# kdexd/virtex

Hardware: NVIDIA H100
Metric: image-caption pairs/sec bicaptioning R50-L1-H1024 (higher is better)
Workload: dtype bf16

## Files before the change

virtex_b200/csrc/gemm_tc.cu:

```cuda
#include <stdlib.h>
#include "ptx.cuh"
#include "vtx_common.cuh"
#include "../../include/virtex_b200.h"

#define KP_TAPS_W p.taps_w
#define KP_PAD p.pad
#define KP_NTAPS p.ntaps

namespace vtx {

constexpr int kBM = 128;
constexpr int kBK = 64;
constexpr int kMaxStages = 8;
constexpr int kABytes = kBM * kBK * 2;
constexpr int kSmemTotal = 232448;
constexpr int kCtrlBytes = 1024;
constexpr int kThreads = 384;
constexpr int kEpiThreads = 256;

struct FastDiv {
  uint32_t mul, shr;
};
__device__ __forceinline__ int fdiv(int x, const FastDiv& f) {
  return f.mul == 0u ? x : (int)(__umulhi((uint32_t)x, f.mul) >> f.shr);
// ... 18 lines not shown
  int bn;
  int a_mn, b_mn;
  int m_tiles, n_tiles, k_splits;
  int kb_total, kb_per_split;
  int mode;
  int cH, cW, cN, cpb;
  int lbw, lbh, lbn;
  int tiles_w, tiles_h;
  int out_f32, atomic, act;
  int stages, stage_bytes;
  int cbytes, nbuf;
  int res_tma;
  float alpha;
  void* D;
  long long ldd;
  const float* bias;
  int bias_pairs;
  const __nv_bfloat16* residual;
  long long ldr;
  const uint8_t* res_mask;
  float* stats;
  int taps_w, pad, ntaps;
  int cstride;
  FastDiv d_mn, d_nt, d_mt, d_tw, d_twh, d_cpb, d_taps;
  unsigned int* sched;
  unsigned int sched_base;
  int sched_chunk;
  int nt_major;
  const __nv_bfloat16* bnr_y;
  const float* bnr_bnp;
  const uint8_t* bnr_mask;
  long long bnr_ldy, bnr_sw, bnr_sh, bnr_sn;
  int vW, vH;
  int bnr_prefetch;
  int bnr;
  int trans_d;
  const float* col_scale;
  const float* col_shift;
};

__device__ __forceinline__ float gelu_erf(float x) { return 0.5f * x * (1.0f + erff(x * 0.70710678118654752f)); }

__device__ __forceinline__ void epi_bar(int id, int threads) {
  asm volatile("bar.sync %0, %1;" ::"r"(id), "r"(threads) : "memory");
}

__device__ __forceinline__ void decode_tile(const GemmKParams& p, int t, int& ks, int& mt, int& nt) {
  ks = fdiv(t, p.d_mn);
  const int rem = t - ks * (p.m_tiles * p.n_tiles);
  if (p.nt_major) {
    nt = fdiv(rem, p.d_mt);
    mt = rem - nt * p.m_tiles;
  } else {
    mt = fdiv(rem, p.d_nt);
    nt = rem - mt * p.n_tiles;
  }
}
__device__ __forceinline__ void tma_prefetch_l2_2d(const void* tmap, int c0, int c1) {
  asm volatile("cp.async.bulk.prefetch.tensor.2d.L2.global.tile [%0, {%1, %2}];" ::"l"(reinterpret_cast<uint64_t>(tmap)),
               "r"(c0), "r"(c1)
               : "memory");
}
__device__ __forceinline__ void tma_prefetch_l2_4d(const void* tmap, int c0, int c1, int c2, int c3) {
  asm volatile("cp.async.bulk.prefetch.tensor.4d.L2.global.tile [%0, {%1, %2, %3, %4}];" ::"l"(
                   reinterpret_cast<uint64_t>(tmap)),
               "r"(c0), "r"(c1), "r"(c2), "r"(c3)
               : "memory");
// ... 248 lines not shown
    }
    epi_bar(bar_id, epi_threads);
    if (et < p.bn && st_nt * p.bn + et < p.N) {
      float a = 0.f, b = 0.f;
      for (int g = 0; g < st_rgs; ++g) {
        const float2 v = *reinterpret_cast<const float2*>(scr + (g * p.bn + et) * 2);
        a += v.x;
        b += v.y;
      }
      if (p.bnr) b *= __ldg(p.bnr_bnp + p.N + st_nt * p.bn + et);
      atomicAdd(p.stats + st_nt * p.bn + et, a);
      atomicAdd(p.stats + p.N + st_nt * p.bn + et, b);
    }
    epi_bar(bar_id, epi_threads);
  };
  auto issue_residual = [&](int t_, int bi_) {
    int ks_, mt_, nt_;
    decode_tile(p, t_, ks_, mt_, nt_);
    const int nb_ = nt_ * p.bn;
    uint8_t* buf_ = cstage0 + (size_t)bi_ * p.cbytes;
    const int slabs = (min(p.bn, p.N - nb_) + 63) >> 6;
    mbar_arrive_expect_tx(&res_bar[bi_], (uint32_t)slabs * 16384u);
    for (int sl = 0; sl < slabs; ++sl) {
      if (p.mode & 1) {
        const int tn_ = fdiv(mt_, p.d_twh);
        const int rwh_ = mt_ - tn_ * (p.tiles_w * p.tiles_h);
        const int th_ = fdiv(rwh_, p.d_tw), tw_ = rwh_ - th_ * p.tiles_w;
        tma_load_4d(buf_ + sl * 16384, &tmR, &res_bar[bi_], nb_ + sl * 64, tw_ << p.lbw, th_ << p.lbh, tn_ << p.lbn);
      } else {
        tma_load_2d(buf_ + sl * 16384, &tmR, &res_bar[bi_], nb_ + sl * 64, mt_ * kBM);
      }
    }
  };
  float acc[NH * BN / 2];
  for (int it = 0;; ++it) {
    const int sit = PP ? 2 * it + wg : it;
    const int slot = sit & (kSched - 1);
    mbar_wait(&sch_full[slot], (sit / kSched) & 1);
    const unsigned long long tk = sch_tile[slot];
    const int t = (int)(uint32_t)tk;
    const int kpos = (int)(tk >> 32);
    mbar_arrive(&sch_empty[slot]);
    if (t >= total_tiles) break;
    int ks, mt, nt;
    decode_tile(p, t, ks, mt, nt);
    const int n_base = nt * p.bn;
    int tw = 0, th = 0, tn = 0;
    if (p.mode & 1) {
      tn = fdiv(mt, p.d_twh);
      const int r_wh = mt - tn * (p.tiles_w * p.tiles_h);
      th = fdiv(r_wh, p.d_tw);
      tw = r_wh - th * p.tiles_w;
    }
    const int cbi = PP ? wg : p.nbuf > 1 ? (it & 1) : 0;
    uint8_t* cbuf = cstage0 + (size_t)cbi * p.cbytes;
    if (staged) {
      if (p.bnr && p.res_tma) epi_bar(bar_id, epi_threads);
      if (et == 0) {
        if (!PP && p.nbuf > 1) tma_store_wait_read<1>();
        else tma_store_wait_read<0>();
      }
      const bool new_block = p.stats != nullptr && st_nt != nt;
      if (new_block && st_nt >= 0 && p.res_tma) {
        epi_bar(bar_id, epi_threads);
        flush_stats(cbuf);
      }
      if (et == 0) {
        if (p.res_tma) issue_residual(t, cbi);
        if (p.bnr && p.bnr_prefetch) {
          const int slabs = (min(p.bn, p.N - n_base) + 63) >> 6;
          for (int sl = 0; sl < slabs; ++sl) {
            if (p.mode & 1) tma_prefetch_l2_4d(&tmY, n_base + sl * 64, tw << p.lbw, th << p.lbh, tn << p.lbn);
            else tma_prefetch_l2_2d(&tmY, n_base + sl * 64, mt * kBM);
          }
        }
      }
      epi_bar(bar_id, epi_threads);
      if (new_block) {
        if (st_nt >= 0 && !p.res_tma) flush_stats(cbuf);
        st_nt = nt;
      }
    }

    {
      const int kb0 = ks * p.kb_per_split;
      const int kb1 = min(p.kb_total, kb0 + p.kb_per_split);
      const int stage = kpos % p.stages;
      const uint32_t phase = (uint32_t)(kpos / p.stages) & 1u;
      const uint32_t a_off = PP ? 0u : (uint32_t)wg * 8192u;
      uint64_t* order_next = nullptr;
      if (PP) {
        if (wg == 1) mbar_wait(&order_bar[1], (uint32_t)it & 1u);
        else if (it > 0) mbar_wait(&order_bar[0], (uint32_t)(it - 1) & 1u);
        order_next = &order_bar[wg ^ 1];
      }
      if (!p.a_mn && !p.b_mn)
        mma_tile<BN, NH, 0, 0>(acc, smem, p, kb0, kb1, a_off, full_bar, empty_bar, stage, phase, signal, order_next);
      else if (!p.a_mn)
        mma_tile<BN, NH, 0, 1>(acc, smem, p, kb0, kb1, a_off, full_bar, empty_bar, stage, phase, signal, order_next);
      else if (!p.b_mn)
        mma_tile<BN, NH, 1, 0>(acc, smem, p, kb0, kb1, a_off, full_bar, empty_bar, stage, phase, signal, order_next);
      else
        mma_tile<BN, NH, 1, 1>(acc, smem, p, kb0, kb1, a_off, full_bar, empty_bar, stage, phase, signal, order_next);
    }
    if (p.res_tma) {
      const int uses = PP ? it : p.nbuf > 1 ? (it >> 1) : it;
      mbar_wait(&res_bar[cbi], uses & 1);
    }
// ... 47 lines not shown
      const uint32_t srow = smem_u32(cbuf) + ((PP ? 0 : wg) * 64 + wl * 16 + (lane >> 2)) * 128 + q * 4;
      const int sw = lane >> 2;
      const int col0 = n_base + 2 * q;
#pragma unroll
      for (int j = 0; j < BN / 8; ++j) {
        const int col = col0 + 8 * j;
        const float2 b = col < p.N ? __ldg(reinterpret_cast<const float2*>(p.bias + col)) : make_float2(0.f, 0.f);
        const uint32_t sa = srow + (j >> 3) * 16384 + (((j & 7) ^ sw) << 4);
#pragma unroll
        for (int hh = 0; hh < 2 * NH; ++hh) {
          const float* accb = acc + (hh >> 1) * (BN / 2) + 4 * j + 2 * (hh & 1);
          sts32(sa + ((hh >> 1) * 64 + 8 * (hh & 1)) * 128, pack_bf16x2(accb[0] + b.x, accb[1] + b.y));
        }
      }
    } else if (plain || p.res_tma) {
#pragma unroll
      for (int hh = 0; hh < 2 * NH; ++hh) {
        const int hr = hh & 1;
        const float* accb = acc + (hh >> 1) * (BN / 2);
        const int r_in_tile = (PP ? (hh >> 1) : wg) * 64 + wl * 16 + (lane >> 2) + 8 * hr;
        const uint32_t srow = smem_u32(cbuf) + r_in_tile * 128 + q * 4;
        const int sw = r_in_tile & 7;
        if (plain) {
#pragma unroll
          for (int j = 0; j < BN / 8; ++j)
            sts32(srow + (j >> 3) * 16384 + (((j & 7) ^ sw) << 4), pack_bf16x2(accb[4 * j + 2 * hr], accb[4 * j + 2 * hr + 1]));
        } else if (p.res_mask == nullptr) {
#pragma unroll
          for (int j = 0; j < BN / 8; ++j) {
            const uint32_t sa = srow + (j >> 3) * 16384 + (((j & 7) ^ sw) << 4);
            sts32(sa, add_res_bf16x2(accb[4 * j + 2 * hr], accb[4 * j + 2 * hr + 1], lds32(sa)));
          }
        } else {
          const long long grow = tile_row(r_in_tile);
          uint32_t mword = 0u;
#pragma unroll
          for (int j = 0; j < BN / 8; ++j) {
            const int col = n_base + 8 * j + 2 * q;
            if ((j & 3) == 0)
              mword = (grow >= 0 && col < p.N)
                          ? __ldg(reinterpret_cast<const uint32_t*>(p.res_mask) + ((grow * p.N + col) >> 5)) : 0u;
            const uint32_t sa = srow + (j >> 3) * 16384 + (((j & 7) ^ sw) << 4);
            const uint32_t r = lds32(sa) & ((((mword >> (col & 31)) & 1u) ? 0x0000ffffu : 0u) |
                                            (((mword >> ((col & 31) + 1)) & 1u) ? 0xffff0000u : 0u));
            sts32(sa, add_res_bf16x2(accb[4 * j + 2 * hr], accb[4 * j + 2 * hr + 1], r));
          }
        }
      }
    } else if (f32_only) {
      float* const D = reinterpret_cast<float*>(p.D);
#pragma unroll
      for (int hh = 0; hh < 2 * NH; ++hh) {
        const int hr = hh & 1;
        const float* accb = acc + (hh >> 1) * (BN / 2);
        const int r_in_tile = (PP ? (hh >> 1) : wg) * 64 + wl * 16 + (lane >> 2) + 8 * hr;
        const long long grow = tile_row(r_in_tile);
        if (grow < 0) continue;
        if (p.trans_d) {
#pragma unroll
          for (int j = 0; j < BN / 8; ++j) {
            const int col = n_base + 8 * j + 2 * q;
            if (col >= p.N) continue;
            float* op = D + (long long)col * p.ldd + grow;
            atomicAdd(op, accb[4 * j + 2 * hr] * p.alpha);
            if (col + 1 < p.N) atomicAdd(op + p.ldd, accb[4 * j + 2 * hr + 1] * p.alpha);
          }
        } else if (p.atomic) {
#pragma unroll
          for (int j = 0; j < BN / 8; ++j) {
            const int col = n_base + 8 * j + 2 * q;
            if (col >= p.N) continue;
            float* op = D + grow * p.ldd + col;
            const float v0 = accb[4 * j + 2 * hr] * p.alpha, v1 = accb[4 * j + 2 * hr + 1] * p.alpha;
            if (col + 1 < p.N) red_add_v2(op, v0, v1);
// ... 50 lines not shown
          if (p.act == 1) {
            v0 = fmaxf(v0, 0.f);
            v1 = fmaxf(v1, 0.f);
          } else if (p.act == 2) {
            v0 = gelu_erf(v0);
            v1 = gelu_erf(v1);
          }
          if (staged) {
            sts32(sa, pack_bf16x2(v0, v1));
          } else if (grow >= 0) {
            float* D = reinterpret_cast<float*>(p.D);
            if (p.trans_d) {
              float* op = D + (long long)col * p.ldd + grow;
              atomicAdd(op, v0);
              if (two) atomicAdd(op + p.ldd, v1);
            } else {
              float* op = D + grow * p.ldd + col;
              if (p.atomic) {
                if (two) red_add_v2(op, v0, v1);
                else atomicAdd(op, v0);
              } else if (two) {
                *reinterpret_cast<float2*>(op) = make_float2(v0, v1);
              } else {
                op[0] = v0;
              }
            }
          }
        }
      }
    }

    const int bnr_r0 = srg * st_rpt;
    const int bnr_col = n_base + scg * 8;
    const bool bnr_on = p.bnr && st_on && bnr_col < p.N;
    auto bnr_load = [&](int rb, uint4* yv, uint32_t& mbits) {
      mbits = 0u;
#pragma unroll
      for (int r4 = 0; r4 < 4; ++r4) {
        const int r = bnr_r0 + rb + r4;
        uint32_t off, lin = 0;
        bool ok;
        if (p.mode & 1) {
          const int dw = r & ((1 << p.lbw) - 1);
          const int dh = (r >> p.lbw) & ((1 << p.lbh) - 1);
          const int dn = r >> (p.lbw + p.lbh);
          const int w = (tw << p.lbw) + dw, h = (th << p.lbh) + dh, n = (tn << p.lbn) + dn;
          ok = (w < p.vW) && (h < p.vH) && (n < p.cN);
          off = (uint32_t)n * (uint32_t)p.bnr_sn + (uint32_t)h * (uint32_t)p.bnr_sh + (uint32_t)w * (uint32_t)p.bnr_sw;
        } else {
          lin = (uint32_t)(mt * kBM + r);
          ok = lin < (uint32_t)p.M;
          off = lin * (uint32_t)p.bnr_ldy;
        }
        yv[r4] = ok ? ldg128_nc(p.bnr_y + off + bnr_col) : make_uint4(0u, 0u, 0u, 0u);
        const uint32_t mw = ok ? (p.bnr == 2 ? (uint32_t)__ldg(p.bnr_mask + ((lin * (uint32_t)p.N + bnr_col) >> 3)) : 0xffu) : 0u;
        mbits |= mw << (8 * r4);
      }
    };

    if (staged) {
      fence_proxy_async();
      epi_bar(bar_id, epi_threads);
      if (et == 0) {
        const int slabs = (min(p.bn, p.N - n_base) + 63) >> 6;
        for (int sl = 0; sl < slabs; ++sl) {
          if (p.mode & 1)
            tma_store_4d(&tmD, cbuf + sl * 16384, n_base + sl * 64, tw << p.lbw, th << p.lbh, tn << p.lbn);
          else
            tma_store_2d(&tmD, cbuf + sl * 16384, n_base + sl * 64, mt * kBM);
        }
        tma_store_commit();
      }
      if (bnr_on) {
        const uint32_t cp = smem_u32(cbuf) + (scg >> 3) * 16384 + bnr_r0 * 128;
        const int c8 = scg & 7;
        float mean[8], sc[8], sh[8];
        {
          const float4 m0 = __ldg(reinterpret_cast<const float4*>(p.bnr_bnp + bnr_col));
          const float4 m1 = __ldg(reinterpret_cast<const float4*>(p.bnr_bnp + bnr_col + 4));
          mean[0] = m0.x; mean[1] = m0.y; mean[2] = m0.z; mean[3] = m0.w;
          mean[4] = m1.x; mean[5] = m1.y; mean[6] = m1.z; mean[7] = m1.w;
          const float4 a0 = __ldg(reinterpret_cast<const float4*>(p.bnr_bnp + 2 * p.N + bnr_col));
          const float4 a1 = __ldg(reinterpret_cast<const float4*>(p.bnr_bnp + 2 * p.N + bnr_col + 4));
          const float4 b0 = __ldg(reinterpret_cast<const float4*>(p.bnr_bnp + 3 * p.N + bnr_col));
          const float4 b1 = __ldg(reinterpret_cast<const float4*>(p.bnr_bnp + 3 * p.N + bnr_col + 4));
          sc[0] = a0.x; sc[1] = a0.y; sc[2] = a0.z; sc[3] = a0.w; sc[4] = a1.x; sc[5] = a1.y; sc[6] = a1.z; sc[7] = a1.w;
          sh[0] = b0.x; sh[1] = b0.y; sh[2] = b0.z; sh[3] = b0.w; sh[4] = b1.x; sh[5] = b1.y; sh[6] = b1.z; sh[7] = b1.w;
        }
        for (int rb = 0; rb < st_rpt; rb += 4) {
          uint4 yv[4];
          uint32_t mbits;
          bnr_load(rb, yv, mbits);
#pragma unroll
          for (int r4 = 0; r4 < 4; ++r4) {
            const int r = rb + r4;
            const uint4 raw = lds128(cp + r * 128 + ((c8 ^ ((bnr_r0 + r) & 7)) << 4));
            float f[8], yy[8];
            unpack8(*reinterpret_cast<const bf16x8*>(&raw), f);
            unpack8(*reinterpret_cast<const bf16x8*>(&yv[r4]), yy);
#pragma unroll
            for (int i = 0; i < 8; ++i) {
              const bool on = p.bnr == 1 ? ((yy[i] * sc[i] + sh[i] > 0.f) && ((mbits >> (8 * r4)) & 0xffu) != 0u)
                                         : (((mbits >> (8 * r4 + i)) & 1u) != 0u);
              const float dz = on ? f[i] : 0.f;
              st_s[i] += dz;
              st_q[i] += dz * (yy[i] - mean[i]);
            }
          }
        }
      }
      if (!p.bnr && p.stats != nullptr && st_on) {
        const int r0 = srg * st_rpt;
        const uint32_t cp = smem_u32(cbuf) + (scg >> 3) * 16384 + r0 * 128;
        const int c8 = scg & 7;
        for (int rb = 0; rb < st_rpt; rb += 4) {
#pragma unroll
          for (int r4 = 0; r4 < 4; ++r4) {
            const int r = rb + r4;
            const uint4 raw = lds128(cp + r * 128 + ((c8 ^ ((r0 + r) & 7)) << 4));
            float f[8];
            unpack8(*reinterpret_cast<const bf16x8*>(&raw), f);
#pragma unroll
            for (int i = 0; i < 8; ++i) {
              st_s[i] += f[i];
              st_q[i] += f[i] * f[i];
            }
          }
        }
      }
    }
  }
  if (staged) {
    if (et == 0) tma_store_wait_read<0>();
    epi_bar(bar_id, epi_threads);
    if (p.stats != nullptr && st_nt >= 0) flush_stats(cstage0 + (PP ? (size_t)wg * p.cbytes : 0));
  }
}

typedef CUresult (*PFN_encodeTiled)(CUtensorMap*, CUtensorMapDataType, cuuint32_t, void*, const cuuint64_t*,
// ... 70 lines not shown

static int ilog2(int x) {
  int l = 0;
  while ((1 << l) < x) ++l;
  return l;
}

static void choose_box(int H, int W, int positions, int* bw, int* bh, int* bn) {
  int best_w = 1, best_h = 1;
  double best_eff = -1;
  for (int w = 1; w <= positions; w <<= 1)
    for (int h = 1; w * h <= positions; h <<= 1) {
      if (w > 2 * W || h > 2 * H) continue;
      const int tw = (W + w - 1) / w, th = (H + h - 1) / h;
      const double eff = (double)(W * H) / ((double)tw * w * th * h);
      const double score = eff * 1000.0 + w * 0.01 + h * 0.0001;
      if (score > best_eff) { best_eff = score; best_w = w; best_h = h; }
    }
  *bw = best_w; *bh = best_h; *bn = positions / (best_w * best_h);
}

template <bool SS>
static cudaError_t launch_gemm(const cudaLaunchConfig_t& cfg, bool pingpong, int bn, const CUtensorMap& tmA,
                               const CUtensorMap& tmB, const CUtensorMap& tmD, const CUtensorMap& tmR,
                               const CUtensorMap& tmY, const GemmKParams& p) {
  if (pingpong && bn == 64) return cudaLaunchKernelEx(&cfg, gemm_wgmma_kernel<64, true, SS>, tmA, tmB, tmD, tmR, tmY, p);
  if (pingpong) return cudaLaunchKernelEx(&cfg, gemm_wgmma_kernel<128, true, SS>, tmA, tmB, tmD, tmR, tmY, p);
  if (bn == 64) return cudaLaunchKernelEx(&cfg, gemm_wgmma_kernel<64, false, SS>, tmA, tmB, tmD, tmR, tmY, p);
  if (bn == 128) return cudaLaunchKernelEx(&cfg, gemm_wgmma_kernel<128, false, SS>, tmA, tmB, tmD, tmR, tmY, p);
  if (bn == 192) return cudaLaunchKernelEx(&cfg, gemm_wgmma_kernel<192, false, SS>, tmA, tmB, tmD, tmR, tmY, p);
  return cudaLaunchKernelEx(&cfg, gemm_wgmma_kernel<256, false, SS>, tmA, tmB, tmD, tmR, tmY, p);
}

}

using namespace vtx;

extern "C" int vtx_gemm_set_dynamic_schedule(int on) {
  g_sched_dynamic = on ? 1 : 0;
  return VTX_OK;
}

extern "C" int vtx_gemm(const VtxGemm* g, void* stream_) {
  cudaStream_t stream = reinterpret_cast<cudaStream_t>(stream_);
  if (!g || !g->A || !g->B || !g->D) return set_error(VTX_EINVAL, "vtx_gemm: null pointer");
  if (g->M <= 0 || g->N <= 0 || g->K <= 0) return set_error(VTX_EINVAL, "vtx_gemm: empty problem");
  if (g->atomic && !g->out_f32) return set_error(VTX_EINVAL, "vtx_gemm: atomic accumulate needs fp32 output");
  if (g->split_k > 1 && !g->atomic) return set_error(VTX_EINVAL, "vtx_gemm: split_k > 1 needs atomic = 1");
  if (g->stats && (g->out_f32 || g->bias || g->residual || g->act || (g->alpha != 0.f && g->alpha != 1.f)))
    return set_error(VTX_EINVAL, "vtx_gemm: stats needs a plain bf16 output (no bias/residual/activation/alpha)");
  if (g->ldd % (g->out_f32 ? 4 : 8) != 0) return set_error(VTX_EINVAL, "vtx_gemm: ldd must keep rows 16B aligned");
  if (g->conv_mode < 0 || g->conv_mode > 6 || g->conv_mode == 3)
    return set_error(VTX_EINVAL, "vtx_gemm: conv_mode must be 0, 1, 2, 4, 5 or 6");
  VtxGemm g4;
  const bool trans_d = g->conv_mode == 4;
  if (trans_d) {
    if (g->conv_c != 64 || g->N != 64 || g->M != 9 * 64 || !g->out_f32 || !g->atomic)
      return set_error(VTX_EINVAL, "vtx_gemm: conv_mode 4 needs C = Cout = 64, M = 576, fp32 atomic output");
    g4 = *g;
    g4.conv_mode = 2;
    g4.M = g->N;
    g4.N = g->M;
    g4.split_k = vtx_num_sms() / 3;
    g4.conv_stride = 1;
    g4.conv_taps = 0;
    g = &g4;
// ... 51 lines not shown
    return set_error(VTX_EINVAL, "vtx_gemm: bad tile_n %d", bn);
  bn = bn <= 64 ? 64 : bn <= 128 ? 128 : bn <= 192 ? 192 : 256;
  const bool pingpong = bn <= 128 && !g->out_f32;
  p.bn = bn;
  p.n_tiles = (g->N + bn - 1) / bn;
  p.trans_d = trans_d ? 1 : 0;
  p.out_f32 = g->out_f32; p.atomic = g->atomic; p.act = g->act;
  p.alpha = g->alpha == 0.f ? 1.0f : g->alpha;
  p.D = g->D; p.ldd = g->ldd;
  p.bias = g->bias;
  p.bias_pairs = (g->bias != nullptr && g->N % 2 == 0 && (reinterpret_cast<uintptr_t>(g->bias) & 7) == 0) ? 1 : 0;
  p.residual = reinterpret_cast<const __nv_bfloat16*>(g->residual);
  p.ldr = g->ldr;
  p.res_mask = reinterpret_cast<const uint8_t*>(g->residual_mask);
  if (p.res_mask != nullptr && (g->residual == nullptr || g->N % 32 != 0 || g->conv_mode != 0 || g->out_f32 ||
                                (reinterpret_cast<uintptr_t>(g->residual_mask) & 3) != 0))
    return set_error(VTX_EINVAL, "vtx_gemm: residual_mask needs a residual, a plain bf16 GEMM and N %% 32 == 0");
  p.stats = g->stats;
  const bool bnr = g->bnr_y != nullptr;
  if (bnr) {
    if (!g->bnr_bnp || !g->bnr_sums || g->stats || g->out_f32 || g->bias || g->act || (g->alpha != 0.f && g->alpha != 1.f) ||
        g->N % 8 != 0 || g->bnr_ldy % 8 != 0 || (reinterpret_cast<uintptr_t>(g->bnr_y) & 15) != 0 ||
        (reinterpret_cast<uintptr_t>(g->bnr_bnp) & 15) != 0 || (g->bnr_mask != nullptr && g->conv_mode != 0) ||
        g->conv_mode == 2 || g->conv_mode >= 4 || split_k > 1)
      return set_error(VTX_EINVAL, "vtx_gemm: bnr needs a plain bf16 output (no stats/bias/activation/alpha/split-K), "
                                   "N %% 8 == 0, 16-byte aligned y / bnp; the bit-mask form needs conv_mode 0");
    if ((long long)g->M * (g->bnr_ldy > g->N ? g->bnr_ldy : g->N) >= (1ll << 31))
      return set_error(VTX_EUNSUPPORTED, "vtx_gemm: bnr needs M * ld(y) < 2^31");
    p.stats = g->bnr_sums;
    p.bnr_y = reinterpret_cast<const __nv_bfloat16*>(g->bnr_y);
    p.bnr_bnp = g->bnr_bnp;
    p.bnr_mask = g->bnr_mask;
    p.bnr_ldy = g->bnr_ldy;
    const char* pf = getenv("VTX_BNR_PREFETCH");
    p.bnr_prefetch = (pf != nullptr && pf[0] == '0') ? 0 : 1;
    p.bnr = g->bnr_mask == nullptr ? 1 : 2;
  }
  const bool ss = g->col_scale != nullptr || g->col_shift != nullptr;
  if (ss) {
    if (!g->col_scale || !g->col_shift || g->out_f32 || (g->alpha != 0.f && g->alpha != 1.f) || g->bias || g->stats ||
        bnr || g->act < 0 || g->act > 1 || g->N % 2 != 0 || (reinterpret_cast<uintptr_t>(g->col_scale) & 7) != 0 ||
        (reinterpret_cast<uintptr_t>(g->col_shift) & 7) != 0 || g->residual_mask || g->conv_out_w > 0 ||
        (g->conv_mode != 0 && g->conv_mode != 1) ||
        (g->residual && (g->ldr % 8 != 0 || (reinterpret_cast<uintptr_t>(g->residual) & 15) != 0)))
      return set_error(VTX_EINVAL, "vtx_gemm: col_scale / col_shift need both vectors 8-byte aligned, a bf16 output, "
                                   "alpha 1, act 0 or 1, N %% 2 == 0, conv_mode 0 or 1 without an output view, no bias / "
                                   "stats / bnr / residual mask, and a 16-byte aligned residual with ldr %% 8 == 0");
    p.col_scale = g->col_scale;
    p.col_shift = g->col_shift;
  }

  CUtensorMap tmA, tmB;
  int rc;
  if (p.mode == 0) {
    p.m_tiles = (g->M + kBM - 1) / kBM;
    p.kb_total = (g->K + kBK - 1) / kBK;
    {
      uint64_t dims[2], str[1];
      uint32_t box[2];
      if (!p.a_mn) { dims[0] = g->K; dims[1] = g->M; box[0] = 64; box[1] = 128; }
      else { dims[0] = g->M; dims[1] = g->K; box[0] = 64; box[1] = 64; }
      str[0] = g->lda;
      if ((rc = make_tmap(&tmA, g->A, 2, dims, str, box)) != VTX_OK) return rc;
    }
    {
      uint64_t dims[2], str[1];
      uint32_t box[2];
      if (!p.b_mn) { dims[0] = g->K; dims[1] = g->N; box[0] = 64; box[1] = (uint32_t)bn; }
      else { dims[0] = g->N; dims[1] = g->K; box[0] = 64; box[1] = 64; }
      str[0] = g->ldb;
// ... 167 lines not shown
```

virtex_b200/engine.py:

```python
from __future__ import annotations

import math
import struct
from typing import Dict, List, Optional, Tuple

import torch
from torch import nn

from . import ops
from .modules import LinearTextualHead
from .ops import call, gemm, _p, _stream

BF16, F32 = torch.bfloat16, torch.float32
_ALIGN = 64
DECODE_MAX_KEYS = 64


def _round_up(x, m):
    return (x + m - 1) // m * m


class Arena:

    def __init__(self, named_params: List[Tuple[str, nn.Parameter]], device):
# ... 53 lines not shown

class _Workspace:

    def __init__(self, device):
        self.device = device
        self.flat: Dict[str, torch.Tensor] = {}

    def get(self, name, shape, dtype):
        shape = tuple(int(s) for s in shape)
        n = 1
        for s in shape:
            n *= s
        t = self.flat.get(name)
        if t is None or t.dtype != dtype or t.numel() < n:
            t = torch.empty(max(n, 1), dtype=dtype, device=self.device)
            self.flat[name] = t
        return t[:n].view(shape)

    def nbytes(self):
        return sum(t.numel() * t.element_size() for t in self.flat.values())


def _require_cuda(dev):
    if dev is None or dev.type != "cuda":
        raise RuntimeError("virtex_b200 has no CPU path: move the model to a CUDA device first (model.cuda())")


def _block_widths(blk):
    return blk.conv1.weight.shape[0], blk.conv3.weight.shape[0]


class Engine:

    fuse_bn3_min_rows = 100000

    def __init__(self, visual=None, textual=None, backward_textual=None, prefix_map=None, ignore_indices=None):
        self.visual, self.textual, self.backward_textual = visual, textual, backward_textual
        named: List[Tuple[str, nn.Parameter]] = []
        if visual is not None:
            named += [("visual." + n, p) for n, p in visual.named_parameters()]
        if textual is not None:
            named += [("textual." + n, p) for n, p in textual.named_parameters()]
        if backward_textual is not None:
            named += [("backward_textual." + n, p) for n, p in backward_textual.named_parameters()]
        dev = None
        for _, p in named:
            dev = p.device
            break
        _require_cuda(dev)
        self.device = dev
        self.arena = Arena(named, dev)
        self.ws = _Workspace(dev)
        self.buffers: Dict[str, torch.Tensor] = {}
        if visual is not None:
            self.buffers.update({"visual." + n: b for n, b in visual.named_buffers()})
        head = textual if textual is not None else backward_textual
        self.pad = getattr(head, "padding_idx", 0) if head is not None else 0
        self.classify = isinstance(textual, LinearTextualHead)
        self.ignore = torch.tensor([int(i) for i in (ignore_indices or [])], dtype=torch.int64, device=dev)
        self._cls = None
        self.seed = torch.zeros(1, dtype=torch.int64, device=dev)
        self.loss = torch.zeros(2, dtype=F32, device=dev)
        self.count = torch.zeros(2, dtype=F32, device=dev)
        self._packed: Dict[str, torch.Tensor] = {}
        self._tape = None
        self.generation = 0
        self._weights_fresh = False
# ... 1162 lines not shown
```

Before: 5871.

## Issue next tile's residual TMA load early and batch residual-mask loads in epilogue

At the end of each tile's epilogue, the epilogue peeks at the next scheduled tile. When double buffering allows, it issues that tile's residual TMA load into the other staging buffer right away. Otherwise it prefetches the residual and mask rows into L2, so the next tile's residual wait overlaps current work. The residual-mask words are now loaded up front for the whole row instead of inside the inner loop. The BN-reduction loop is restructured with a compile-time row count, and the env-controlled prefetch switch is removed. This adds an extra scheduler wait per tile and more registers, and the modified compile-time row bound could mismatch st_rpt.

```diff
diff --git a/virtex_b200/csrc/gemm_tc.cu b/virtex_b200/csrc/gemm_tc.cu
--- a/virtex_b200/csrc/gemm_tc.cu
+++ b/virtex_b200/csrc/gemm_tc.cu
@@ -74,7 +74,6 @@
   const uint8_t* bnr_mask;
   long long bnr_ldy, bnr_sw, bnr_sh, bnr_sn;
   int vW, vH;
-  int bnr_prefetch;
   int bnr;
   int trans_d;
   const float* col_scale;
@@ -389,6 +388,21 @@
       }
     }
   };
+  auto prefetch_tile_l2 = [&](const CUtensorMap* tm, int mt_, int nb_) {
+    const int slabs = (min(p.bn, p.N - nb_) + 63) >> 6;
+    int tw_ = 0, th_ = 0, tn_ = 0;
+    if (p.mode & 1) {
+      tn_ = fdiv(mt_, p.d_twh);
+      const int rwh_ = mt_ - tn_ * (p.tiles_w * p.tiles_h);
+      th_ = fdiv(rwh_, p.d_tw);
+      tw_ = rwh_ - th_ * p.tiles_w;
+    }
+    for (int sl = 0; sl < slabs; ++sl) {
+      if (p.mode & 1) tma_prefetch_l2_4d(tm, nb_ + sl * 64, tw_ << p.lbw, th_ << p.lbh, tn_ << p.lbn);
+      else tma_prefetch_l2_2d(tm, nb_ + sl * 64, mt_ * kBM);
+    }
+  };
+  bool ahead = false, res_ahead = false;
   float acc[NH * BN / 2];
   for (int it = 0;; ++it) {
     const int sit = PP ? 2 * it + wg : it;
@@ -423,14 +437,8 @@
         flush_stats(cbuf);
       }
       if (et == 0) {
-        if (p.res_tma) issue_residual(t, cbi);
-        if (p.bnr && p.bnr_prefetch) {
-          const int slabs = (min(p.bn, p.N - n_base) + 63) >> 6;
-          for (int sl = 0; sl < slabs; ++sl) {
-            if (p.mode & 1) tma_prefetch_l2_4d(&tmY, n_base + sl * 64, tw << p.lbw, th << p.lbh, tn << p.lbn);
-            else tma_prefetch_l2_2d(&tmY, n_base + sl * 64, mt * kBM);
-          }
-        }
+        if (p.res_tma && !res_ahead) issue_residual(t, cbi);
+        if (p.bnr) prefetch_tile_l2(&tmY, mt, n_base);
       }
       epi_bar(bar_id, epi_threads);
       if (new_block) {
@@ -544,14 +552,19 @@
             sts32(sa, add_res_bf16x2(accb[4 * j + 2 * hr], accb[4 * j + 2 * hr + 1], lds32(sa)));
           }
         } else {
-          const long long grow = tile_row(r_in_tile);
-          uint32_t mword = 0u;
+          const int r_ = mt * kBM + r_in_tile;
+          uint32_t mwords[BN / 32];
+#pragma unroll
+          for (int c = 0; c < BN / 32; ++c) {
+            const int col = n_base + 32 * c + 2 * q;
+            mwords[c] = (r_ < p.M && col < p.N)
+                            ? __ldg(reinterpret_cast<const uint32_t*>(p.res_mask) + (((long long)r_ * p.N + col) >> 5))
+                            : 0u;
+          }
 #pragma unroll
           for (int j = 0; j < BN / 8; ++j) {
             const int col = n_base + 8 * j + 2 * q;
-            if ((j & 3) == 0)
-              mword = (grow >= 0 && col < p.N)
-                          ? __ldg(reinterpret_cast<const uint32_t*>(p.res_mask) + ((grow * p.N + col) >> 5)) : 0u;
+            const uint32_t mword = mwords[j >> 2];
             const uint32_t sa = srow + (j >> 3) * 16384 + (((j & 7) ^ sw) << 4);
             const uint32_t r = lds32(sa) & ((((mword >> (col & 31)) & 1u) ? 0x0000ffffu : 0u) |
                                             (((mword >> ((col & 31) + 1)) & 1u) ? 0xffff0000u : 0u));
@@ -668,7 +681,7 @@
 
     const int bnr_r0 = srg * st_rpt;
     const int bnr_col = n_base + scg * 8;
-    const bool bnr_on = p.bnr && st_on && bnr_col < p.N;
+    const bool bnr_on = !SS && p.bnr && st_on && bnr_col < p.N;
     auto bnr_load = [&](int rb, uint4* yv, uint32_t& mbits) {
       mbits = 0u;
 #pragma unroll
@@ -707,7 +720,35 @@
         }
         tma_store_commit();
       }
+      if constexpr (!PP && !SS) {
+        if (p.res_tma) {
+          const int nsit = sit + 1;
+          const int nslot = nsit & (kSched - 1);
+          mbar_wait(&sch_full[nslot], (nsit / kSched) & 1);
+          const int tnx = (int)(uint32_t)sch_tile[nslot];
+          ahead = tnx < total_tiles;
+          res_ahead = false;
+          if (ahead) {
+            int ksx, mtx, ntx;
+            decode_tile(p, tnx, ksx, mtx, ntx);
+            const int mrow = mtx * kBM + et;
+            if (p.res_mask != nullptr && et < 128 && mrow < p.M)
+              asm volatile("prefetch.global.L2 [%0];" ::"l"(p.res_mask + (((long long)mrow * p.N + ntx * p.bn) >> 3)));
+            if (et == 0) {
+              res_ahead = p.res_tma && p.nbuf > 1 && (p.stats == nullptr || ntx == nt);
+              if (res_ahead) {
+                tma_store_wait_read<1>();
+                issue_residual(tnx, (it + 1) & 1);
+              } else if (p.res_tma) {
+                prefetch_tile_l2(&tmR, mtx, ntx * p.bn);
+              }
+            }
+          }
+        }
+      }
       if (bnr_on) {
+        constexpr int kLg = BN == 64 ? 3 : BN == 128 ? 4 : 5;
+        constexpr int kRows = 128 / ((epi_threads >> kLg) < 32 ? (epi_threads >> kLg) : 32);
         const uint32_t cp = smem_u32(cbuf) + (scg >> 3) * 16384 + bnr_r0 * 128;
         const int c8 = scg & 7;
         float mean[8], sc[8], sh[8];
@@ -723,24 +764,30 @@
           sc[0] = a0.x; sc[1] = a0.y; sc[2] = a0.z; sc[3] = a0.w; sc[4] = a1.x; sc[5] = a1.y; sc[6] = a1.z; sc[7] = a1.w;
           sh[0] = b0.x; sh[1] = b0.y; sh[2] = b0.z; sh[3] = b0.w; sh[4] = b1.x; sh[5] = b1.y; sh[6] = b1.z; sh[7] = b1.w;
         }
-        for (int rb = 0; rb < st_rpt; rb += 4) {
-          uint4 yv[4];
-          uint32_t mbits;
-          bnr_load(rb, yv, mbits);
-#pragma unroll
-          for (int r4 = 0; r4 < 4; ++r4) {
-            const int r = rb + r4;
-            const uint4 raw = lds128(cp + r * 128 + ((c8 ^ ((bnr_r0 + r) & 7)) << 4));
-            float f[8], yy[8];
-            unpack8(*reinterpret_cast<const bf16x8*>(&raw), f);
-            unpack8(*reinterpret_cast<const bf16x8*>(&yv[r4]), yy);
-#pragma unroll
-            for (int i = 0; i < 8; ++i) {
-              const bool on = p.bnr == 1 ? ((yy[i] * sc[i] + sh[i] > 0.f) && ((mbits >> (8 * r4)) & 0xffu) != 0u)
-                                         : (((mbits >> (8 * r4 + i)) & 1u) != 0u);
-              const float dz = on ? f[i] : 0.f;
-              st_s[i] += dz;
-              st_q[i] += dz * (yy[i] - mean[i]);
+        constexpr int kB = 4;
+        for (int r8 = 0; r8 < kRows; r8 += kB) {
+          uint4 yv[kB];
+          uint32_t mbits[kB / 4];
+#pragma unroll
+          for (int b = 0; b < kB / 4; ++b) bnr_load(r8 + 4 * b, yv + 4 * b, mbits[b]);
+#pragma unroll
+          for (int rb = 0; rb < kB; rb += 4) {
+            const uint32_t mb = mbits[rb >> 2];
+#pragma unroll
+            for (int r4 = 0; r4 < 4; ++r4) {
+              const int r = rb + r4;
+              const uint4 raw = lds128(cp + (r8 + r) * 128 + ((c8 ^ ((bnr_r0 + r8 + r) & 7)) << 4));
+              float f[8], yy[8];
+              unpack8(*reinterpret_cast<const bf16x8*>(&raw), f);
+              unpack8(*reinterpret_cast<const bf16x8*>(&yv[r]), yy);
+#pragma unroll
+              for (int i = 0; i < 8; ++i) {
+                const bool on = p.bnr == 1 ? ((yy[i] * sc[i] + sh[i] > 0.f) && ((mb >> (8 * r4)) & 0xffu) != 0u)
+                                           : (((mb >> (8 * r4 + i)) & 1u) != 0u);
+                const float dz = on ? f[i] : 0.f;
+                st_s[i] += dz;
+                st_q[i] += dz * (yy[i] - mean[i]);
+              }
             }
           }
         }
@@ -994,8 +1041,6 @@
     p.bnr_bnp = g->bnr_bnp;
     p.bnr_mask = g->bnr_mask;
     p.bnr_ldy = g->bnr_ldy;
-    const char* pf = getenv("VTX_BNR_PREFETCH");
-    p.bnr_prefetch = (pf != nullptr && pf[0] == '0') ? 0 : 1;
     p.bnr = g->bnr_mask == nullptr ? 1 : 2;
   }
   const bool ss = g->col_scale != nullptr || g->col_shift != nullptr;
```

After: 5888 (median of 6 runs). Within noise of the previous version (+0.3%).

## Add specialized small-K residual dgrad GEMM kernel with fused masked residual and BN stats

Applied to the files above, without the earlier changes.

Adds a dedicated warp-specialized WGMMA kernel for residual-masked backward GEMMs with K of 64, 128 or 256. It keeps the weight tile resident in shared memory and streams 64-row A, residual and mask tiles through a TMA pipeline. The epilogue fuses the masked residual add and, optionally, the BN-backward reductions (sum and centered dot product). It is dispatched automatically from vtx_gemm when the shape fits, and the fuse_bn3 row threshold is lowered so more layers take the fused path. This trades a new code path and persistent-walker scheduling for less redundant reloading of A and W and fewer separate passes.

```diff
diff --git a/virtex_b200/csrc/gemm_resid.cu b/virtex_b200/csrc/gemm_resid.cu
--- /dev/null
+++ b/virtex_b200/csrc/gemm_resid.cu
@@ -0,0 +1,369 @@
+#include "ptx.cuh"
+#include "vtx_common.cuh"
+#include "../../include/virtex_b200.h"
+
+namespace vtx {
+
+namespace {
+
+constexpr int kRBM = 64;
+constexpr int kRMaxStages = 8;
+constexpr int kRThreads = 288;
+constexpr int kRSmem = 232448;
+constexpr int kRCtrl = 1024;
+constexpr int kRMaskBytes = kRBM * 16;
+
+struct ResidParams {
+  int m_tiles, walkers, nblk;
+  int stages, stage_bytes, a_bytes;
+  int N;
+  const float* bnp;
+  float* sums;
+};
+
+__device__ __forceinline__ uint32_t res_add(float lo, float hi, uint32_t res) {
+  const __nv_bfloat162 o = __hadd2(__floats2bfloat162_rn(lo, hi), *reinterpret_cast<const __nv_bfloat162*>(&res));
+  return *reinterpret_cast<const uint32_t*>(&o);
+}
+__device__ __forceinline__ uint32_t lds32r(uint32_t a) {
+  uint32_t v;
+  asm volatile("ld.shared.b32 %0, [%1];" : "=r"(v) : "r"(a));
+  return v;
+}
+__device__ __forceinline__ void sts32r(uint32_t a, uint32_t v) {
+  asm volatile("st.shared.b32 [%0], %1;" ::"r"(a), "r"(v) : "memory");
+}
+__device__ __forceinline__ void named_bar(int id, int threads) {
+  asm volatile("bar.sync %0, %1;" ::"r"(id), "r"(threads) : "memory");
+}
+__device__ __forceinline__ uint32_t keep_halves(uint32_t w, uint32_t bits) {
+  return w & (((bits & 1u) ? 0x0000ffffu : 0u) | ((bits & 2u) ? 0xffff0000u : 0u));
+}
+
+template <bool BNR, int KB, int BN>
+__global__ void __launch_bounds__(kRThreads, 1)
+resid_dgrad_kernel(const __grid_constant__ CUtensorMap tmA, const __grid_constant__ CUtensorMap tmW,
+                   const __grid_constant__ CUtensorMap tmR, const __grid_constant__ CUtensorMap tmM,
+                   const __grid_constant__ CUtensorMap tmY, const __grid_constant__ CUtensorMap tmMB,
+                   const __grid_constant__ CUtensorMap tmD, const ResidParams p) {
+  VTX_PDL_TRIGGER();
+  extern __shared__ uint8_t smem_raw[];
+  uint8_t* base = reinterpret_cast<uint8_t*>((reinterpret_cast<uintptr_t>(smem_raw) + 1023) & ~uintptr_t(1023));
+  uint64_t* full_bar = reinterpret_cast<uint64_t*>(base);
+  uint64_t* empty_bar = full_bar + kRMaxStages;
+  uint64_t* w_bar = empty_bar + kRMaxStages;
+  float* s_mean = reinterpret_cast<float*>(base + 512);
+  constexpr int NS = BN / 64;
+  constexpr int kOutBytes = kRBM * BN * 2;
+  uint8_t* sW = base + kRCtrl;
+  uint8_t* sOut = sW + KB * NS * 8192;
+  uint8_t* sStage = sOut + 2 * kOutBytes;
+
+  const int warp = __shfl_sync(0xffffffffu, (int)(threadIdx.x >> 5), 0);
+  const int lane = threadIdx.x & 31;
+  const int nb = blockIdx.x % p.nblk;
+  const int wk = blockIdx.x / p.nblk;
+  const int mask_off = p.a_bytes + NS * 8192 + (BNR ? NS * 8192 : 0);
+
+  if (warp == 8 && lane == 0) {
+    tma_prefetch_desc(&tmA);
+    tma_prefetch_desc(&tmW);
+    tma_prefetch_desc(&tmR);
+    tma_prefetch_desc(&tmM);
+    tma_prefetch_desc(&tmD);
+    if (BNR) {
+      tma_prefetch_desc(&tmY);
+      tma_prefetch_desc(&tmMB);
+    }
+    for (int i = 0; i < p.stages; ++i) {
+      mbar_init(&full_bar[i], 1);
+      mbar_init(&empty_bar[i], 1);
+    }
+    mbar_init(w_bar, 1);
+    fence_mbar_init();
+  }
+  __syncthreads();
+  VTX_PDL_WAIT();
+
+  if (warp == 8) {
+    if (lane == 0) {
+      mbar_arrive_expect_tx(w_bar, (uint32_t)(KB * NS * 8192));
+      for (int kb = 0; kb < KB; ++kb)
+        for (int j = 0; j < NS; ++j) tma_load_2d(sW + (kb * NS + j) * 8192, &tmW, w_bar, nb * BN + 64 * j, kb * 64);
+      const uint32_t tx = (uint32_t)(p.a_bytes + NS * 8192 + kRMaskBytes + (BNR ? NS * 8192 + kRMaskBytes : 0));
+      int s = 0;
+      for (int mt = wk; mt < p.m_tiles; mt += p.walkers, ++s) {
+        const int stage = s % p.stages;
+        mbar_wait(&empty_bar[stage], ((uint32_t)(s / p.stages) & 1u) ^ 1u);
+        uint8_t* st = sStage + stage * p.stage_bytes;
+        uint64_t* fb = &full_bar[stage];
+        mbar_arrive_expect_tx(fb, tx);
+        const int r0 = mt * kRBM, c0 = nb * BN, mc0 = (c0 / 128) * 16;
+        for (int kb = 0; kb < KB; ++kb) tma_load_2d(st + kb * 8192, &tmA, fb, kb * 64, r0);
+        for (int j = 0; j < NS; ++j) tma_load_2d(st + p.a_bytes + j * 8192, &tmR, fb, c0 + 64 * j, r0);
+        tma_load_2d(st + mask_off, &tmM, fb, mc0, r0);
+        if (BNR) {
+          for (int j = 0; j < NS; ++j) tma_load_2d(st + p.a_bytes + (NS + j) * 8192, &tmY, fb, c0 + 64 * j, r0);
+          tma_load_2d(st + mask_off + kRMaskBytes, &tmMB, fb, mc0, r0);
+        }
+      }
+    }
+    return;
+  }
+
+  const int ct = threadIdx.x;
+  const int wg = ct >> 7;
+  const int wl = (ct >> 5) & 3;
+  const int t = ct & 127;
+  const int q = lane & 3;
+  const int sw = lane >> 2;
+  if (BNR) {
+    if (ct < BN) s_mean[ct] = __ldg(p.bnp + nb * BN + ct);
+    named_bar(3, 256);
+  }
+  constexpr int NP = BNR ? BN / 4 : 1;
+  float ps[NP], pq[NP];
+#pragma unroll
+  for (int i = 0; i < NP; ++i) ps[i] = pq[i] = 0.f;
+
+  uint8_t* out = sOut + wg * kOutBytes;
+  const uint32_t sW0 = smem_u32(sW);
+  mbar_wait(w_bar, 0);
+  for (int s = wg;; s += 2) {
+    const int mt = wk + s * p.walkers;
+    if (mt >= p.m_tiles) break;
+    const int stage = s % p.stages;
+    const int round = s / p.stages;
+    if (round > 0) mbar_wait(&empty_bar[stage], (uint32_t)(round - 1) & 1u);
+    mbar_wait(&full_bar[stage], (uint32_t)round & 1u);
+    const uint32_t st = smem_u32(sStage + stage * p.stage_bytes);
+
+    float acc[BN / 2];
+#pragma unroll
+    for (int i = 0; i < BN / 2; ++i) fence_operand(acc[i]);
+    wgmma_fence();
+#pragma unroll
+    for (int kb = 0; kb < KB; ++kb) {
+#pragma unroll
+      for (int k = 0; k < 4; ++k) {
+        const uint64_t ad = make_wgmma_desc(st + kb * 8192 + k * 32, 16, 1024);
+        const uint64_t bd = make_wgmma_desc(sW0 + kb * NS * 8192 + k * 2048, 8192, 1024);
+        if constexpr (BN == 128) wgmma_n128<0, 1>(acc, ad, bd, (kb > 0 || k > 0) ? 1u : 0u);
+        else wgmma_n64<0, 1>(acc, ad, bd, (kb > 0 || k > 0) ? 1u : 0u);
+      }
+    }
+    wgmma_commit();
+    wgmma_wait<0>();
+#pragma unroll
+    for (int i = 0; i < BN / 2; ++i) fence_operand(acc[i]);
+
+    if (t == 0) tma_store_wait_read<0>();
+    named_bar(1 + wg, 128);
+
+    uint32_t m3[2][BN / 32], mb[2][BN / 32];
+    const bool upper = BN == 64 && (nb & 1);
+#pragma unroll
+    for (int hh = 0; hh < 2; ++hh) {
+      const int r = wl * 16 + sw + 8 * hh;
+      const uint4 v = lds128(st + mask_off + r * 16);
+      m3[hh][0] = upper ? v.z : v.x; m3[hh][1] = upper ? v.w : v.y;
+      if (BN == 128) { m3[hh][BN / 64] = v.z; m3[hh][BN / 32 - 1] = v.w; }
+      if (BNR) {
+        const uint4 b = lds128(st + mask_off + kRMaskBytes + r * 16);
+        mb[hh][0] = upper ? b.z : b.x; mb[hh][1] = upper ? b.w : b.y;
+        if (BN == 128) { mb[hh][BN / 64] = b.z; mb[hh][BN / 32 - 1] = b.w; }
+      }
+    }
+    const uint32_t row0 = (uint32_t)(wl * 16 + sw) * 128 + q * 4;
+    const uint32_t so = smem_u32(out);
+#pragma unroll
+    for (int j = 0; j < BN / 8; ++j) {
+      const uint32_t off = row0 + (j >> 3) * 8192 + (((j & 7) ^ sw) << 4);
+      const int bit = 8 * (j & 3) + 2 * q;
+      float2 mean = make_float2(0.f, 0.f);
+      if (BNR) mean = *reinterpret_cast<const float2*>(s_mean + 8 * j + 2 * q);
+#pragma unroll
+      for (int hh = 0; hh < 2; ++hh) {
+        const uint32_t a = off + hh * 8 * 128;
+        const uint32_t res = keep_halves(lds32r(st + p.a_bytes + a), m3[hh][j >> 2] >> bit);
+        const uint32_t o = res_add(acc[4 * j + 2 * hh], acc[4 * j + 2 * hh + 1], res);
+        sts32r(so + a, o);
+        if (BNR) {
+          const uint32_t dz = keep_halves(o, mb[hh][j >> 2] >> bit);
+          const uint32_t y = lds32r(st + p.a_bytes + NS * 8192 + a);
+          const float dz0 = __uint_as_float(dz << 16), dz1 = __uint_as_float(dz & 0xffff0000u);
+          ps[2 * j] += dz0;
+          ps[2 * j + 1] += dz1;
+          pq[2 * j] += dz0 * (__uint_as_float(y << 16) - mean.x);
+          pq[2 * j + 1] += dz1 * (__uint_as_float(y & 0xffff0000u) - mean.y);
+        }
+      }
+    }
+    fence_proxy_async();
+    named_bar(1 + wg, 128);
+    if (t == 0) {
+      mbar_arrive(&empty_bar[stage]);
+      for (int j = 0; j < NS; ++j) tma_store_2d(&tmD, out + j * 8192, nb * BN + 64 * j, mt * kRBM);
+      tma_store_commit();
+    }
+  }
+  if (t == 0) tma_store_wait_read<0>();
+  if (BNR) {
+#pragma unroll
+    for (int i = 0; i < NP; ++i) {
+#pragma unroll
+      for (int o = 4; o < 32; o <<= 1) {
+        ps[i] += __shfl_xor_sync(0xffffffffu, ps[i], o);
+        pq[i] += __shfl_xor_sync(0xffffffffu, pq[i], o);
+      }
+    }
+    named_bar(3, 256);
+    float2* scr = reinterpret_cast<float2*>(sOut);
+    if (sw == 0) {
+#pragma unroll
+      for (int j = 0; j < BN / 8; ++j) {
+        scr[warp * BN + 8 * j + 2 * q] = make_float2(ps[2 * j], pq[2 * j]);
+        scr[warp * BN + 8 * j + 2 * q + 1] = make_float2(ps[2 * j + 1], pq[2 * j + 1]);
+      }
+    }
+    named_bar(3, 256);
+    if (ct < BN) {
+      float a = 0.f, b = 0.f;
+      for (int w = 0; w < 8; ++w) {
+        const float2 v = scr[w * BN + ct];
+        a += v.x;
+        b += v.y;
+      }
+      const int col = nb * BN + ct;
+      atomicAdd(p.sums + col, a);
+      atomicAdd(p.sums + p.N + col, b * __ldg(p.bnp + p.N + col));
+    }
+  }
+}
+
+typedef CUresult (*PFN_encode)(CUtensorMap*, CUtensorMapDataType, cuuint32_t, void*, const cuuint64_t*,
+                               const cuuint64_t*, const cuuint32_t*, const cuuint32_t*, CUtensorMapInterleave,
+                               CUtensorMapSwizzle, CUtensorMapL2promotion, CUtensorMapFloatOOBfill);
+
+int tmap2d(CUtensorMap* tm, const void* ptr, bool bytes, uint64_t cols, uint64_t rows, uint64_t ld, uint32_t box_c,
+           uint32_t box_r) {
+  static PFN_encode enc = nullptr;
+  if (enc == nullptr) {
+    void* fp = nullptr;
+    cudaDriverEntryPointQueryResult qr;
+    if (cudaGetDriverEntryPoint("cuTensorMapEncodeTiled", &fp, cudaEnableDefault, &qr) != cudaSuccess ||
+        qr != cudaDriverEntryPointSuccess)
+      return set_error(VTX_ECUDA, "cuTensorMapEncodeTiled entry point not available");
+    enc = reinterpret_cast<PFN_encode>(fp);
+  }
+  const cuuint64_t dims[2] = {cols, rows};
+  const cuuint64_t str[1] = {ld * (bytes ? 1 : 2)};
+  const cuuint32_t box[2] = {box_c, box_r};
+  const cuuint32_t es[2] = {1, 1};
+  const CUresult r = enc(tm, bytes ? CU_TENSOR_MAP_DATA_TYPE_UINT8 : CU_TENSOR_MAP_DATA_TYPE_BFLOAT16, 2,
+                         const_cast<void*>(ptr), dims, str, box, es, CU_TENSOR_MAP_INTERLEAVE_NONE,
+                         bytes ? CU_TENSOR_MAP_SWIZZLE_NONE : CU_TENSOR_MAP_SWIZZLE_128B,
+                         CU_TENSOR_MAP_L2_PROMOTION_L2_256B, CU_TENSOR_MAP_FLOAT_OOB_FILL_NONE);
+  if (r != CUDA_SUCCESS) return set_error(VTX_ECUDA, "cuTensorMapEncodeTiled failed (%d)", (int)r);
+  return VTX_OK;
+}
+
+bool al16(const void* p) { return (reinterpret_cast<uintptr_t>(p) & 15) == 0; }
+
+int resid_bn(const VtxGemm* g) { return g->K > 128 ? 64 : 128; }
+int resid_stage_bytes(const VtxGemm* g) {
+  const bool bnr = g->bnr_y != nullptr;
+  const int slabs = resid_bn(g) / 64;
+  return (g->K / 64) * 8192 + slabs * 8192 + kRMaskBytes + (bnr ? slabs * 8192 + kRMaskBytes : 0);
+}
+int resid_stages(const VtxGemm* g) {
+  const int bn = resid_bn(g);
+  const int fixed = 1024  + kRCtrl + (g->K / 64) * (bn / 64) * 8192 + 2 * kRBM * bn * 2;
+  const int st = (kRSmem - fixed) / resid_stage_bytes(g);
+  return st < 3 ? 0 : st > kRMaxStages ? kRMaxStages : st;
+}
+
+template <bool BNR, int KB, int BN>
+cudaError_t launch_resid(const cudaLaunchConfig_t& cfg, const CUtensorMap& tmA, const CUtensorMap& tmW,
+                         const CUtensorMap& tmR, const CUtensorMap& tmM, const CUtensorMap& tmY,
+                         const CUtensorMap& tmMB, const CUtensorMap& tmD, const ResidParams& p) {
+  cudaError_t e = cudaFuncSetAttribute(resid_dgrad_kernel<BNR, KB, BN>, cudaFuncAttributeMaxDynamicSharedMemorySize,
+                                       kRSmem);
+  if (e != cudaSuccess) return e;
+  return cudaLaunchKernelEx(&cfg, resid_dgrad_kernel<BNR, KB, BN>, tmA, tmW, tmR, tmM, tmY, tmMB, tmD, p);
+}
+
+}
+
+bool resid_dgrad_serves(const VtxGemm* g) {
+  const bool bnr = g->bnr_y != nullptr;
+  if (g->conv_mode != 0 || g->a_mn || !g->b_mn || g->out_f32 || g->atomic || g->split_k > 1 || g->act || g->bias ||
+      g->stats || (g->alpha != 0.f && g->alpha != 1.f) || g->col_scale || g->col_shift)
+    return false;
+  if (!g->residual || !g->residual_mask || g->N % 128 != 0 || (g->K != 64 && g->K != 128 && g->K != 256) ||
+      resid_stages(g) == 0)
+    return false;
+  if (g->lda % 8 || g->ldb % 8 || g->ldd % 8 || g->ldr % 8 || !al16(g->A) || !al16(g->B) || !al16(g->D) ||
+      !al16(g->residual) || !al16(g->residual_mask))
+    return false;
+  if (bnr && (!g->bnr_mask || !g->bnr_bnp || !g->bnr_sums || g->bnr_ldy % 8 || !al16(g->bnr_y) || !al16(g->bnr_mask)))
+    return false;
+  return true;
+}
+
+int resid_dgrad(const VtxGemm* g, cudaStream_t stream) {
+  const bool bnr = g->bnr_y != nullptr;
+  const int bn = resid_bn(g);
+  const uint64_t M = (uint64_t)g->M, N = (uint64_t)g->N, K = (uint64_t)g->K;
+  CUtensorMap tmA, tmW, tmR, tmM, tmY, tmMB, tmD;
+  memset(&tmY, 0, sizeof(tmY));
+  memset(&tmMB, 0, sizeof(tmMB));
+  int rc;
+  if ((rc = tmap2d(&tmA, g->A, false, K, M, (uint64_t)g->lda, 64, kRBM)) != VTX_OK) return rc;
+  if ((rc = tmap2d(&tmW, g->B, false, N, K, (uint64_t)g->ldb, 64, 64)) != VTX_OK) return rc;
+  if ((rc = tmap2d(&tmR, g->residual, false, N, M, (uint64_t)g->ldr, 64, kRBM)) != VTX_OK) return rc;
+  if ((rc = tmap2d(&tmM, g->residual_mask, true, N / 8, M, N / 8, 16, kRBM)) != VTX_OK) return rc;
+  if ((rc = tmap2d(&tmD, g->D, false, N, M, (uint64_t)g->ldd, 64, kRBM)) != VTX_OK) return rc;
+  if (bnr) {
+    if ((rc = tmap2d(&tmY, g->bnr_y, false, N, M, (uint64_t)g->bnr_ldy, 64, kRBM)) != VTX_OK) return rc;
+    if ((rc = tmap2d(&tmMB, g->bnr_mask, true, N / 8, M, N / 8, 16, kRBM)) != VTX_OK) return rc;
+  }
+  ResidParams p;
+  memset(&p, 0, sizeof(p));
+  p.m_tiles = (g->M + kRBM - 1) / kRBM;
+  p.nblk = g->N / bn;
+  const int kb = g->K / 64;
+  p.a_bytes = kb * 8192;
+  p.stage_bytes = resid_stage_bytes(g);
+  p.stages = resid_stages(g);
+  p.N = g->N;
+  p.bnp = g->bnr_bnp;
+  p.sums = g->bnr_sums;
+  const int sms = vtx_num_sms();
+  int walkers = sms / p.nblk;
+  if (walkers < 1) walkers = 1;
+  if (walkers > p.m_tiles) walkers = p.m_tiles;
+  p.walkers = walkers;
+  cudaLaunchConfig_t cfg;
+  memset(&cfg, 0, sizeof(cfg));
+  cfg.gridDim = dim3((unsigned)(walkers * p.nblk));
+  cfg.blockDim = dim3(kRThreads);
+  cfg.dynamicSmemBytes = kRSmem;
+  cfg.stream = stream;
+  cudaLaunchAttribute attr[1];
+  attr[0].id = cudaLaunchAttributeProgrammaticStreamSerialization;
+  attr[0].val.programmaticStreamSerializationAllowed = 1;
+  cfg.attrs = attr;
+  cfg.numAttrs = 1;
+  cudaError_t le;
+  if (kb == 1) le = bnr ? launch_resid<true, 1, 128>(cfg, tmA, tmW, tmR, tmM, tmY, tmMB, tmD, p)
+                        : launch_resid<false, 1, 128>(cfg, tmA, tmW, tmR, tmM, tmY, tmMB, tmD, p);
+  else if (kb == 2) le = bnr ? launch_resid<true, 2, 128>(cfg, tmA, tmW, tmR, tmM, tmY, tmMB, tmD, p)
+                             : launch_resid<false, 2, 128>(cfg, tmA, tmW, tmR, tmM, tmY, tmMB, tmD, p);
+  else le = bnr ? launch_resid<true, 4, 64>(cfg, tmA, tmW, tmR, tmM, tmY, tmMB, tmD, p)
+                : launch_resid<false, 4, 64>(cfg, tmA, tmW, tmR, tmM, tmY, tmMB, tmD, p);
+  if (le != cudaSuccess) return set_error(VTX_ECUDA, "resid_dgrad_kernel launch: %s", cudaGetErrorString(le));
+  return VTX_OK;
+}
+
+}
diff --git a/virtex_b200/csrc/gemm_tc.cu b/virtex_b200/csrc/gemm_tc.cu
--- a/virtex_b200/csrc/gemm_tc.cu
+++ b/virtex_b200/csrc/gemm_tc.cu
@@ -877,6 +877,9 @@
   return cudaLaunchKernelEx(&cfg, gemm_wgmma_kernel<256, false, SS>, tmA, tmB, tmD, tmR, tmY, p);
 }
 
+bool resid_dgrad_serves(const VtxGemm* g);
+int resid_dgrad(const VtxGemm* g, cudaStream_t stream);
+
 }
 
 using namespace vtx;
@@ -998,6 +1001,7 @@
     p.bnr_prefetch = (pf != nullptr && pf[0] == '0') ? 0 : 1;
     p.bnr = g->bnr_mask == nullptr ? 1 : 2;
   }
+  if (g->tile_n == 0 && resid_dgrad_serves(g)) return resid_dgrad(g, stream);
   const bool ss = g->col_scale != nullptr || g->col_shift != nullptr;
   if (ss) {
     if (!g->col_scale || !g->col_shift || g->out_f32 || (g->alpha != 0.f && g->alpha != 1.f) || g->bias || g->stats ||
diff --git a/virtex_b200/engine.py b/virtex_b200/engine.py
--- a/virtex_b200/engine.py
+++ b/virtex_b200/engine.py
@@ -109,7 +109,7 @@
 
 class Engine:
 
-    fuse_bn3_min_rows = 100000
+    fuse_bn3_min_rows = 40000
 
     def __init__(self, visual=None, textual=None, backward_textual=None, prefix_map=None, ignore_indices=None):
         self.visual, self.textual, self.backward_textual = visual, textual, backward_textual
```

Result: faster. 5917 before, 6108 after (median of 6 runs) (+3.2%).
